# KamilSJaron/smudgeplot

Hardware: NVIDIA H100
Metric: k-mers/sec scanned (hetmers) at 1/2/4/8 H100; bit-exact .smu vs ref C (higher is better)
Workload: dtype u64

## Files before the change

smudgeplot_b200/csrc/hm_symm.cu:

```cuda
#include <cuda_runtime.h>
#include <stdint.h>
#include <stdio.h>
#include <stdlib.h>
#include <string.h>

#include "hetmers_b200.h"
#include "hm_internal.h"
#include "hm_device.cuh"

#define RS_THREADS 256
#define RS_EPT     8
#define RS_TILE    (RS_THREADS*RS_EPT)
#define RS_HALO    64
#define RS_WIN     (RS_TILE+2*RS_HALO)
#define RS_SCANCAP RS_HALO
#define RS_RUNCAP  (RS_HALO+1)
#define RS_LONGRUN 32
#ifndef RS_MINBLOCKS
#define RS_MINBLOCKS 5
#endif
#ifndef RS_STAGE
#define RS_STAGE   384
#endif

#define SY_STATUS_ASYMMETRIC 1ull
#define SY_STATUS_OVERFLOW   2ull

#define SY_HDR_CAND   0
#define SY_HDR_STATUS 1
#define SY_HDR_RUNS   2
#define SY_HDR_S      3
#define SY_HDR_PEND   4
#define SY_HDR_QUERY  5

struct SymmView
  { unsigned long long *cand_n;
    unsigned long long *status;
    uint32_t *bloom;
    uint32_t  seg_words;
    int       n_seg, self;
    uint64_t  first_key[HM_MAX_SHARDS];
    uint64_t *cand_key, *cand_lo, *cand_meta;
    unsigned long long cand_cap;
    unsigned long long *runs_n;
    uint64_t *runs;
    unsigned long long runs_cap;
    uint64_t *s_key, *s_lo;
    unsigned long long s_cap;
    const hm_stream_sview *sviews;
    uint64_t *pend, *pend_key, *pend_lo;
    uint64_t *q_key, *q_lo, *q_tag;
    unsigned long long pend_cap, q_cap;
  };

template <int KW>
__device__ __forceinline__ void bloom_slot(const SymmView &W, int seg, int kmer, uint64_t hi, uint64_t lo,
                                           uint32_t *&word, uint32_t &mask)
{ const int Pr = kmer >> 1, pup = kmer-Pr;
  uint64_t sfx;
  if (KW == 1)
    sfx = hi >> (64-2*kmer);
  else
    { const int sr = 128-2*kmer;
      sfx = sr == 0 ? lo : ((lo >> sr) | (hi << (64-sr)));
    }
  if (2*Pr < 64)
    sfx &= (((uint64_t) 1 << (2*Pr)) - 1);
  const uint64_t pfx = hi >> (64-2*pup);
  uint32_t h = ((uint32_t) sfx ^ (uint32_t) (sfx >> 32) * 0x85EBCA6Bu) * 0x9E3779B1u;
  uint32_t g = ((uint32_t) pfx ^ (uint32_t) (pfx >> 32) * 0xC2B2AE35u) * 0x27D4EB2Fu;
  h ^= h >> 15;
  word = W.bloom + (size_t) seg * W.seg_words + __umulhi(h * 0x2C1B3C6Du,W.seg_words);
  mask = (1u << (g >> 27)) | (1u << ((g >> 22) & 31));
}

__device__ __forceinline__ uint32_t ld_keep(const uint32_t *p)
{ uint32_t v; uint64_t pol;
  asm volatile("createpolicy.fractional.L2::evict_last.b64 %0, 1.0;" : "=l"(pol));
  asm volatile("ld.global.nc.L1::no_allocate.L2::cache_hint.u32 %0, [%1], %2;" : "=r"(v) : "l"(p), "l"(pol));
  return v;
}

__device__ __forceinline__ uint64_t ld_stream(const uint64_t *p)
{ uint64_t v, pol;
  asm volatile("createpolicy.fractional.L2::evict_first.b64 %0, 1.0;" : "=l"(pol));
  asm volatile("ld.global.nc.L1::no_allocate.L2::cache_hint.u64 %0, [%1], %2;" : "=l"(v) : "l"(p), "l"(pol));
  return v;
}

__device__ __forceinline__ int owner_of(const SymmView &W, uint64_t hi)
{ int r = 0;
  for (int s = 1; s < W.n_seg; s++)
    r += (hi >= W.first_key[s]);
  return r;
}

template <typename IdxT, int KW>
__device__ __noinline__ void neighbours_slow(const uint64_t *__restrict__ keys, const uint64_t *__restrict__ keys_lo,
                                             const uint16_t *__restrict__ cnt, const IdxT *__restrict__ bucket,
                                             int bshift, int kmer, int p0, int pup,
                                             uint64_t x, uint64_t xl, int cx,
                                             int &H, int &U, int64_t &part, int &ppos)
{ H = 0; U = 0; part = -1; ppos = 0;
  for (int p = p0; p < kmer; p++)
    { int b = base_at<KW>(x,xl,p);
      for (int c = 0; c < 4; c++)
        { if (c == b) continue;
          uint64_t y = x, yl = xl;
          set_base<KW>(y,yl,p,c);
          int64_t j = bucket_find<IdxT,KW>(keys,keys_lo,bucket,bshift,y,yl);
          if (j >= 0 && cx + (int) __ldg(cnt+j) <= HM_SMAX)
            { H += 1;
              if (p >= pup) U += 1;
              part = j; ppos = p;
            }
        }
    }
}


__device__ __forceinline__ uint64_t fp_mix(uint64_t hi, uint64_t lo, uint32_t c, uint64_t seed)
{ uint64_t v = (hi ^ seed) * 0xBF58476D1CE4E5B9ull;
  v ^= v >> 32;
  v = (v + lo + ((uint64_t) c << 40) + c) * 0x94D049BB133111EBull;
  v ^= v >> 29;
  v *= (seed | 1);
  v ^= v >> 32;
  return v;
}

template <int KW>
__global__ void __launch_bounds__(256)
symm_fingerprint_kernel(const uint64_t *__restrict__ keys, const uint64_t *__restrict__ keys_lo,
                        const uint16_t *__restrict__ cnt, int64_t i0, int64_t i1, int kmer,
                        uint64_t seed0, uint64_t seed1, unsigned long long *__restrict__ acc)
{ uint64_t a0 = 0, a1 = 0, a2 = 0, a3 = 0;
// ... 79 lines not shown
  out->off_cand_meta = at;  at += 8*cap;
  out->cand_cap = cap;
  out->off_runs = at;       out->runs_cap = range/3 + 1024;   at += 8*out->runs_cap;
  out->n_seg = n_seg;
  out->range = range;
  out->bytes = (at+255) & ~255ll;
  return HM_OK;
}

static void bloom_window(cudaStream_t st, const void *base, size_t bytes, int on)
{ static int limit_set[64] = {0};
  static size_t max_win[64] = {0}, max_persist[64] = {0};
  int dev = 0;
  cudaGetDevice(&dev);
  if (dev < 0 || dev >= 64) return;
  if (!limit_set[dev])
    { cudaDeviceProp p;
      limit_set[dev] = 1;
      if (cudaGetDeviceProperties(&p,dev) == cudaSuccess)
        { max_win[dev] = (size_t) p.accessPolicyMaxWindowSize;
          max_persist[dev] = (size_t) p.persistingL2CacheMaxSize;
          if (max_persist[dev] > 0)
            cudaDeviceSetLimit(cudaLimitPersistingL2CacheSize,max_persist[dev]);
        }
      cudaGetLastError();
    }
  if (max_win[dev] == 0 || max_persist[dev] == 0)
    return;
  cudaStreamAttrValue a;
  memset(&a,0,sizeof(a));
  if (on)
    { size_t w = bytes < max_win[dev] ? bytes : max_win[dev];
      a.accessPolicyWindow.base_ptr  = (void *) base;
      a.accessPolicyWindow.num_bytes = w;
      a.accessPolicyWindow.hitRatio  = w <= max_persist[dev] ? 1.0f : (float) max_persist[dev] / (float) w;
      a.accessPolicyWindow.hitProp   = cudaAccessPropertyPersisting;
      a.accessPolicyWindow.missProp  = cudaAccessPropertyStreaming;
    }
  cudaStreamSetAttribute(st,cudaStreamAttributeAccessPolicyWindow,&a);
  cudaGetLastError();
}

static int l2_persist(void)
{ const char *e = getenv("HETMERS_L2_PERSIST");
  return (e == NULL || strcmp(e,"0") != 0);
}

static SymmView make_view(void *d_work, const hm_symm_layout *L, const hm_symm_shards *sh)
{ SymmView W;
  uint8_t *b = (uint8_t *) d_work;
  memset(&W,0,sizeof(W));
  W.cand_n    = (unsigned long long *) (b + L->off_header) + SY_HDR_CAND;
  W.status    = W.cand_n + SY_HDR_STATUS;
  W.bloom     = (uint32_t *) (b + L->off_bloom);
  W.seg_words = (uint32_t) L->seg_words;
  W.n_seg     = L->n_seg;
  W.self      = 0;
  if (sh != NULL && sh->n_seg > 1)
    { W.self = sh->self;
      for (int r = 0; r < sh->n_seg; r++) W.first_key[r] = sh->first_key[r];
    }
  W.cand_key  = (uint64_t *) (b + L->off_cand_key);
  W.cand_lo   = (uint64_t *) (b + L->off_cand_lo);
  W.cand_meta = (uint64_t *) (b + L->off_cand_meta);
  W.cand_cap  = (unsigned long long) L->cand_cap;
  W.runs_n    = W.cand_n + SY_HDR_RUNS;
  W.runs      = (uint64_t *) (b + L->off_runs);
  W.runs_cap  = (unsigned long long) L->runs_cap;
  return W;
}


template <int KW> struct RsSmem
  { uint64_t *key, *klo;
    uint16_t *cnt;
    uint64_t *ckey, *clo, *cmeta;
    uint16_t *t1;
    uint16_t *t2r;
  };

__device__ __forceinline__ uint64_t pack_meta(int cx, int cy, int pos, int yb)
{ return (uint64_t) cx | ((uint64_t) cy << 16) | ((uint64_t) pos << 32) | ((uint64_t) yb << 40); }

template <int KW>
__device__ __forceinline__ void stage_candidates(const RsSmem<KW> &S, unsigned *s_nc, const SymmView &W,
                                                 bool emit, uint64_t x, uint64_t xl, uint64_t meta,
                                                 int lane, unsigned lt)
{ const unsigned bal = __ballot_sync(0xffffffffu,emit);
  if (bal == 0)
    return;
  unsigned base = 0;
  if (lane == 0)
    base = atomicAdd(s_nc,(unsigned) __popc(bal));
  base = __shfl_sync(0xffffffffu,base,0);
  const unsigned at = base + __popc(bal & lt);
  const bool     over = emit && (at >= RS_STAGE);
  if (emit && !over)
    { S.ckey[at] = x;
      if (KW == 2) S.clo[at] = xl;
      S.cmeta[at] = meta;
    }
  if (base + __popc(bal) <= RS_STAGE)
    return;
  const unsigned ob = __ballot_sync(0xffffffffu,over);
  unsigned long long g0 = 0;
  if (lane == 0)
    g0 = atomicAdd(W.cand_n,(unsigned long long) __popc(ob));
  g0 = __shfl_sync(0xffffffffu,g0,0) + (unsigned long long) __popc(ob & lt);
  if (over)
    { if (g0 < W.cand_cap)
        { W.cand_key[g0] = x;
          if (KW == 2) W.cand_lo[g0] = xl;
          W.cand_meta[g0] = meta;
        }
      else
        atomicOr(W.status,SY_STATUS_OVERFLOW);
    }
}

template <int KW>
__device__ __forceinline__ void s_push(const SymmView &W, uint64_t x, uint64_t xl)
{ const unsigned m = __activemask();
  const int      lane = threadIdx.x & 31, lead = __ffs(m)-1;
  unsigned long long at = 0;
  if (lane == lead)
    at = atomicAdd(W.cand_n + SY_HDR_S,(unsigned long long) __popc(m));
  at = __shfl_sync(m,at,lead) + (unsigned long long) __popc(m & ((1u << lane)-1));
  if (at < W.s_cap)
    { W.s_key[at] = x;
      if (KW == 2) W.s_lo[at] = xl;
    }
  else
    atomicOr(W.status,SY_STATUS_OVERFLOW);
}

template <int KW, bool SL>
__device__ __forceinline__ void bloom_insert(const SymmView &W, int kmer, uint64_t x, uint64_t xl)
{ uint32_t *word, mask;
  bloom_slot<KW>(W,W.self,kmer,x,xl,word,mask);
  atomicOr(word,mask);
  if (SL)
    s_push<KW>(W,x,xl);
}

template <typename IdxT, int KW, bool SL>
__global__ void __launch_bounds__(256)
runs_kernel(const uint64_t *__restrict__ keys, const uint64_t *__restrict__ keys_lo,
            const uint16_t *__restrict__ cnt, int64_t n, const IdxT *__restrict__ bucket, int bshift,
            int kmer, int64_t lo, int64_t hi, const SymmView W)
{ const int      Pr = kmer >> 1, pup = kmer-Pr, psh = 64-2*Pr;
  const uint64_t pmask = ~(uint64_t) 0 << psh;
  const unsigned FULL = 0xffffffffu;
  const int      lane = threadIdx.x & 31;
  const unsigned lt   = (1u << lane) - 1;
  unsigned long long nrl = *W.runs_n;
  if (nrl > W.runs_cap) nrl = W.runs_cap;
  const int64_t nr     = (int64_t) nrl;
  const int64_t stride = (int64_t) gridDim.x * blockDim.x;
  for (int64_t r0 = (int64_t) blockIdx.x * blockDim.x + threadIdx.x - lane; r0 < nr; r0 += stride)
    { const int64_t r = r0+lane;
      const bool    valid = (r < nr);
      int64_t  h = 0;
      uint64_t x0 = 0;
      if (valid)
        { h  = (int64_t) W.runs[r];
          x0 = __ldg(keys+h);
        }
      unsigned lb = __ballot_sync(FULL,valid);
      while (lb != 0)
        { const int     src = __ffs(lb)-1;
          lb &= lb-1;
          const int64_t hh = __shfl_sync(FULL,h,src);
          const uint64_t xx = __shfl_sync(FULL,x0,src);
          int64_t end = hh+1;
          while (true)
            { const int64_t t = end+lane;
              const bool same = (t < n) && (((__ldg(keys+t) ^ xx) & pmask) == 0);
              const unsigned sb = __ballot_sync(FULL,same);
              if (sb == FULL) { end += 32; continue; }
              end += __ffs(~sb)-1;
              break;
            }
          for (int64_t g0 = hh; g0 < end; g0 += 32)
            { const int64_t g = g0+lane;
              bool     emit = false;
              uint64_t x = 0, xl = 0, meta = 0;
              if (g < end && g >= lo && g < hi)
                { x = __ldg(keys+g);
                  if (KW == 2) xl = __ldg(keys_lo+g);
                  const int cx = __ldg(cnt+g);
                  int Hn, Un, ppos; int64_t part;
                  neighbours_slow<IdxT,KW>(keys,keys_lo,cnt,bucket,bshift,kmer,Pr,pup,x,xl,cx,Hn,Un,part,ppos);
                  if (Un > 0)
                    bloom_insert<KW,SL>(W,kmer,x,xl);
                  if (Hn == 1 && part > g)
                    { const uint64_t y = __ldg(keys+part), yl = KW == 2 ? __ldg(keys_lo+part) : 0;
                      const int cy = __ldg(cnt+part);
                      int Hy, Uy, py; int64_t party;
                      neighbours_slow<IdxT,KW>(keys,keys_lo,cnt,bucket,bshift,kmer,Pr,pup,y,yl,cy,Hy,Uy,party,py);
                      if (Hy == 1)
                        { emit = true;
                          meta = pack_meta(cx,cy,ppos,base_at<KW>(y,yl,ppos));
                        }
                    }
                }
              const unsigned eb = __ballot_sync(FULL,emit);
              if (eb != 0)
                { unsigned long long base = 0;
                  if (lane == 0)
                    base = atomicAdd(W.cand_n,(unsigned long long) __popc(eb));
                  base = __shfl_sync(FULL,base,0) + (unsigned long long) __popc(eb & lt);
                  if (emit)
                    { if (base < W.cand_cap)
                        { W.cand_key[base] = x;
                          if (KW == 2) W.cand_lo[base] = xl;
                          W.cand_meta[base] = meta;
                        }
                      else
                        atomicOr(W.status,SY_STATUS_OVERFLOW);
                    }
                }
            }
        }
    }
}
// ... 18 lines not shown
}

template <int KW, bool SL, int LMAX>
__device__ __forceinline__ bool settle_members(const RsSmem<KW> &S, const SymmView &W, int kmer, int Pr, int pup,
                                               int h, int L, int a, bool in, bool own, int lane,
                                               uint64_t &x, uint64_t &xl, uint64_t &meta)
{ int Hx = 0, Ux = 0, part = 0, ppos = 0, cx = 0;
  if (in)
    { x  = S.key[h+a];
      xl = KW == 2 ? S.klo[h+a] : 0;
      cx = S.cnt[h+a];
      auto mate = [&](int b)
        { int pos;
          if (b < L && b != a && one_base_in_run(run_sfx<KW>(x ^ S.key[h+b],KW == 2 ? xl ^ S.klo[h+b] : 0,Pr),Pr,pos) &&
              cx + (int) S.cnt[h+b] <= HM_SMAX)
            { Hx += 1;
              if (pos >= pup) Ux += 1;
              part = b; ppos = pos;
            }
        };
      if constexpr (LMAX > 0)
        {
#pragma unroll
          for (int b = 0; b < LMAX; b++)
            mate(b);
        }
      else
        for (int b = 0; b < L; b++)
          mate(b);
      if (own && Ux > 0)
        bloom_insert<KW,SL>(W,kmer,x,xl);
    }
  const int pl = lane + part - a;
  int       Hy = __shfl_sync(0xffffffffu,Hx,pl & 31);
  if (!in || !own || Hx != 1 || part < a)
    return false;
  const uint64_t y = S.key[h+part], yl = KW == 2 ? S.klo[h+part] : 0;
  const int      cy = S.cnt[h+part];
  if (pl > 31)
    { Hy = 0;
      for (int b = 0; b < L; b++)
        { int pos;
          if (b != part && one_base_in_run(run_sfx<KW>(y ^ S.key[h+b],KW == 2 ? yl ^ S.klo[h+b] : 0,Pr),Pr,pos) &&
              cy + (int) S.cnt[h+b] <= HM_SMAX)
            Hy += 1;
        }
    }
  if (Hy != 1)
    return false;
  meta = pack_meta(cx,cy,ppos,base_at<KW>(y,yl,ppos));
  return true;
}

#ifdef RS_PROBE
#define RS_PHASES 6
#define RS_PROBE_SLOTS 1024
__device__ unsigned long long rs_probe_cycles[RS_PROBE_SLOTS*RS_PHASES];
__device__ int rs_probe_mode;
#define RS_PROBE_TILE(b)  (rs_probe_mode == 2 ? (b) % 64 : (b))
#define RS_PROBE_START    long long rs_t = clock64(); unsigned long long rs_acc[RS_PHASES] = {0, 0, 0, 0, 0, 0};
#define RS_PROBE_MARK(ph) { const long long t_ = clock64(); rs_acc[ph] += (unsigned long long) (t_ - rs_t); rs_t = t_; }
#define RS_PROBE_FLUSH()  { if (lane == 0) _Pragma("unroll") for (int p_ = 0; p_ < RS_PHASES; p_++) \
                              atomicAdd(rs_probe_cycles + (blockIdx.x % RS_PROBE_SLOTS)*RS_PHASES + p_,rs_acc[p_]); }
#define RS_PROBE_LOADONLY() if (rs_probe_mode == 1) { RS_PROBE_FLUSH(); return; }

extern "C" int hm_probe_runscan(int mode, unsigned long long *cycles)
{ static unsigned long long rows[RS_PROBE_SLOTS*RS_PHASES];
  cudaError_t e = cudaDeviceSynchronize();
  if (e == cudaSuccess && cycles != NULL)
    { e = cudaMemcpyFromSymbol(rows,rs_probe_cycles,sizeof(rows));
      for (int p = 0; p < RS_PHASES; p++)
        { cycles[p] = 0;
          for (int r = 0; r < RS_PROBE_SLOTS; r++)
            cycles[p] += rows[r*RS_PHASES+p];
        }
    }
  memset(rows,0,sizeof(rows));
  if (e == cudaSuccess)
    e = cudaMemcpyToSymbol(rs_probe_cycles,rows,sizeof(rows));
  if (e == cudaSuccess)
    e = cudaMemcpyToSymbol(rs_probe_mode,&mode,sizeof(mode));
  return e == cudaSuccess ? HM_OK : hm_cuda_fail(e,"hm_probe_runscan");
}
#else
#define RS_PROBE_TILE(b)  (b)
#define RS_PROBE_START
#define RS_PROBE_MARK(ph)
#define RS_PROBE_FLUSH()
#define RS_PROBE_LOADONLY()
#endif

template <typename IdxT, int KW, bool SL>
__global__ void __launch_bounds__(RS_THREADS,RS_MINBLOCKS)
runscan_kernel(const uint64_t *__restrict__ keys, const uint64_t *__restrict__ keys_lo,
               const uint16_t *__restrict__ cnt, int64_t n, const IdxT *__restrict__ bucket, int bshift,
               int kmer, int64_t lo, int64_t hi, int64_t tile0, int use_tma, const SymmView W)
{ extern __shared__ __align__(128) uint8_t smem[];
  __shared__ __align__(8) uint64_t s_bar;
  __shared__ unsigned s_nc, s_nr, s_done;
  RsSmem<KW> S;
  S.key   = (uint64_t *) smem;
  S.klo   = S.key + (KW == 2 ? RS_WIN : 0);
  S.ckey  = S.key + KW*RS_WIN;
  S.clo   = S.ckey + (KW == 2 ? RS_STAGE : 0);
  S.cmeta = S.ckey + KW*RS_STAGE;
  S.cnt   = (uint16_t *) (S.cmeta + RS_STAGE);
  S.t1    = S.cnt + RS_WIN;
  S.t2r   = S.t1 + RS_TILE/2;

  const int      Pr   = kmer >> 1;
  const int      pup  = kmer - Pr;
  const int      psh  = 64-2*Pr;
  const uint64_t pmask = ~(uint64_t) 0 << psh;
  const unsigned FULL = 0xffffffffu;
  const int      lane = threadIdx.x & 31;
  const int      warp = threadIdx.x >> 5;
  const unsigned lt   = (1u << lane) - 1;
  RS_PROBE_START

  const int64_t T0 = (tile0 + RS_PROBE_TILE(blockIdx.x)) * RS_TILE;
  const int64_t ws = T0 - RS_HALO;
  const int64_t e0 = ws > 0 ? ws : 0;
  const int64_t e1 = T0+RS_TILE+RS_HALO < n ? T0+RS_TILE+RS_HALO : n;
  const int     v0 = (int) (e0-ws), v1 = (int) (e1-ws);

  const int m   = v1-v0;
  const int mt  = use_tma ? (m & ~7) : 0;
  if (threadIdx.x == 0)
    { s_nc = 0; s_nr = 0; s_done = 0;
      if (mt > 0)
        { mbar_init(&s_bar,1);
          fence_proxy_async_smem();
        }
    }
  __syncthreads();
  if (threadIdx.x == 0 && mt > 0)
    { mbar_arrive_expect_tx(&s_bar,(unsigned) (mt*(8*KW+2)));
      bulk_copy_g2s(S.key+v0,keys+e0,(unsigned) (8*mt),&s_bar);
      if (KW == 2)
        bulk_copy_g2s(S.klo+v0,keys_lo+e0,(unsigned) (8*mt),&s_bar);
      bulk_copy_g2s(S.cnt+v0,cnt+e0,(unsigned) (2*mt),&s_bar);
    }
  if (mt < m || v0 > 0 || v1 < RS_WIN)
    { for (int j = mt + threadIdx.x; j < m; j += RS_THREADS)
        { S.key[v0+j] = keys[e0+j];
          if (KW == 2) S.klo[v0+j] = keys_lo[e0+j];
          S.cnt[v0+j] = cnt[e0+j];
        }
      if (mt > 0)
        mbar_wait(&s_bar,0);
      __syncthreads();
      const uint64_t sa = ~S.key[v0], sb = ~S.key[v1-1];
      __syncthreads();
      for (int j = threadIdx.x; j < RS_WIN; j += RS_THREADS)
        if (j < v0)       S.key[j] = sa;
        else if (j >= v1) S.key[j] = sb;
      __syncthreads();
    }
  else
    mbar_wait(&s_bar,0);
  RS_PROBE_MARK(0)
  RS_PROBE_LOADONLY()

  const int wd0 = RS_HALO/32 + warp*RS_EPT;
  unsigned  eqw = 0;
#pragma unroll
  for (int t = 0; t < RS_EPT+2; t++)
    { const int i = (wd0-1+t)*32 + lane;
      bool eq;
      if (psh >= 32)
        { const uint32_t a = (uint32_t) (S.key[i] >> 32);
          uint32_t       b = __shfl_down_sync(FULL,a,1);
          if (lane == 31) b = (uint32_t) (S.key[i+1] >> 32);
          eq = (((a ^ b) >> (psh-32)) == 0);
        }
      else
        eq = (((S.key[i] ^ S.key[i+1]) & pmask) == 0);
      const unsigned bal = __ballot_sync(FULL,eq);
      if (lane == t) eqw = bal;
    }
  RS_PROBE_MARK(1)

  const int a0 = RS_HALO + (lo > T0 ? (int) (lo-T0 < RS_TILE ? lo-T0 : RS_TILE) : 0);
  const int a1 = RS_HALO + (hi-T0 < RS_TILE ? (int) (hi-T0) : RS_TILE);
  uint16_t *my1  = S.t1  + warp*(RS_TILE/2/(RS_THREADS/32));
  int n1, n3;
  { const unsigned P = __shfl_up_sync(FULL,eqw,1), N = __shfl_down_sync(FULL,eqw,1);
    unsigned m2 = 0, m3 = 0;
    const int wd = wd0-1+lane;
    if (lane >= 1 && lane <= RS_EPT)
      { const unsigned E = eqw;
        const unsigned em1 = (E << 1) | (P >> 31);
        const unsigned em2 = (E << 2) | (P >> 30);
        const unsigned ep1 = (E >> 1) | (N << 31);
        const int      s0  = wd*32;
        unsigned act = 0xffffffffu;
        if (s0 < a0)      act &= (a0-s0 >= 32) ? 0u : (0xffffffffu << (a0-s0));
        if (s0+32 > a1)   act &= (a1-s0 <= 0)  ? 0u : (0xffffffffu >> (s0+32-a1));
        const unsigned more = (em1 & E) | (E & ep1) | (em1 & em2);
        m2 = (E & ~em1 & ~ep1) & act;
        m3 = more & act & ~em1;
      }
    const int c2 = __popc(m2), c3 = __popc(m3);
    int pre2 = c2, pre3 = c3;
#pragma unroll
    for (int o = 1; o <= RS_EPT; o <<= 1)
      { int v2 = __shfl_up_sync(FULL,pre2,o), v3 = __shfl_up_sync(FULL,pre3,o);
        if (lane >= o) { pre2 += v2; pre3 += v3; }
      }
    n1 = __shfl_sync(FULL,pre2,RS_EPT);
    n3 = __shfl_sync(FULL,pre3,RS_EPT);
    int at = pre2-c2;
    while (m2 != 0)
      { my1[at++] = (uint16_t) (wd*32 + __ffs(m2)-1);
        m2 &= m2-1;
      }
    at = n1 + pre3-c3;
    while (m3 != 0)
      { my1[at++] = (uint16_t) (wd*32 + __ffs(m3)-1);
        m3 &= m3-1;
      }
  }
  __syncwarp();
  RS_PROBE_MARK(2)

  for (int i0 = 0; i0 < n1; i0 += 32)
    { const int i = i0+lane;
      bool     emit = false;
      uint64_t x = 0, xl = 0, meta = 0;
      if (i < n1)
        { const int w = my1[i];
          x = S.key[w];
          const uint64_t y = S.key[w+1];
          uint64_t yl = 0;
          if (KW == 2) { xl = S.klo[w]; yl = S.klo[w+1]; }
          const int cx = S.cnt[w], cy = S.cnt[w+1];
          int pos;
          if (one_base_in_run(run_sfx<KW>(x ^ y,xl ^ yl,Pr),Pr,pos) && cx+cy <= HM_SMAX)
            { emit = true;
              meta = pack_meta(cx,cy,pos,base_at<KW>(y,yl,pos));
              if (pos >= pup)
                { bloom_insert<KW,SL>(W,kmer,x,xl);
                  bloom_insert<KW,SL>(W,kmer,y,yl);
                }
            }
        }
      stage_candidates<KW>(S,&s_nc,W,emit,x,xl,meta,lane,lt);
    }
  RS_PROBE_MARK(3)

  const int b1 = hi-T0 < RS_TILE+RS_HALO ? RS_HALO + (int) (hi-T0) : RS_WIN;
  for (int i0 = 0; i0 < n3; i0 += 32)
    { const int i = i0+lane;
      const int h = i < n3 ? my1[n1+i] : 0;
      int       L = 0;
      {
        const int      t  = (h >> 5) - (wd0-1);
        const unsigned w0 = __shfl_sync(FULL,eqw,t & 31), w1 = __shfl_sync(FULL,eqw,(t+1) & 31);
        const unsigned up = __funnelshift_r(w0,w1,h & 31);
        if (i < n3)
          L = (~up != 0) ? __ffs((int) ~up) : 33;
      }
      const int Ls = L <= 8 ? L : 0;
      int inc = Ls;
#pragma unroll
      for (int o = 1; o < 32; o <<= 1)
        { const int v = __shfl_up_sync(FULL,inc,o);
          if (lane >= o) inc += v;
        }
      const int M = __shfl_sync(FULL,inc,31);
      for (int t0 = 0; t0 < M; t0 += 32)
        { const int t = t0+lane;
          int r = 0;
#pragma unroll
          for (int s = 16; s > 0; s >>= 1)
            if (__shfl_sync(FULL,inc,r+s-1) <= t) r += s;
          const int hr = __shfl_sync(FULL,h,r), Lr = __shfl_sync(FULL,Ls,r);
          const int a  = t - (__shfl_sync(FULL,inc,r) - Lr);
          bool     emit = false;
          uint64_t x = 0, xl = 0, meta = 0;
          emit = settle_members<KW,SL,8>(S,W,kmer,Pr,pup,hr,Lr,a,t < M,hr+a < b1,lane,x,xl,meta);
          stage_candidates<KW>(S,&s_nc,W,emit,x,xl,meta,lane,lt);
        }
      unsigned lb = __ballot_sync(FULL,L > 8);
      while (lb != 0)
        { const int src = __ffs(lb)-1;
          lb &= lb-1;
          const int hh = __shfl_sync(FULL,h,src);
          int       LL = __shfl_sync(FULL,L,src);
          if (LL > 32)
            { const uint64_t xh = S.key[hh];
              while (LL <= RS_RUNCAP)
                { const int      t = hh+LL+lane;
                  const unsigned sb = __ballot_sync(FULL,t < RS_WIN && ((S.key[t] ^ xh) & pmask) == 0);
                  if (sb != FULL) { LL += __ffs(~sb)-1; break; }
                  LL += 32;
                }
            }
          if (LL > RS_RUNCAP || hh+LL >= RS_WIN)
            { if (lane == 0)
                S.t2r[atomicAdd(&s_nr,1u)] = (uint16_t) hh;
              continue;
            }
          for (int a0 = 0; a0 < LL; a0 += 32)
            { const int a = a0+lane;
              bool     emit = false;
              uint64_t x = 0, xl = 0, meta = 0;
              emit = settle_members<KW,SL,0>(S,W,kmer,Pr,pup,hh,LL,a,a < LL,hh+a < b1,lane,x,xl,meta);
              stage_candidates<KW>(S,&s_nc,W,emit,x,xl,meta,lane,lt);
            }
        }
    }
  RS_PROBE_MARK(4)

  __syncwarp();
  unsigned last = 0;
  if (lane == 0)
    { __threadfence_block();
      last = (atomicAdd(&s_done,1u) == RS_THREADS/32-1);
    }
  last = __shfl_sync(FULL,last,0);
  if (!last)
    { RS_PROBE_MARK(5) RS_PROBE_FLUSH() return; }
  __threadfence_block();
  const unsigned nr = s_nr;
  if (nr > 0)
    { unsigned long long rb = 0;
      if (lane == 0)
        rb = atomicAdd(W.runs_n,(unsigned long long) nr);
      rb = __shfl_sync(FULL,rb,0);
      for (unsigned i = lane; i < nr; i += 32)
        if (rb+i < W.runs_cap)
          W.runs[rb+i] = (uint64_t) (T0 + ((int) S.t2r[i] - RS_HALO));
        else
          atomicOr(W.status,SY_STATUS_OVERFLOW);
    }
  const unsigned nc = s_nc < RS_STAGE ? s_nc : RS_STAGE;
  if (nc == 0)
    { RS_PROBE_MARK(5) RS_PROBE_FLUSH() return; }
  unsigned long long base = 0;
  if (lane == 0)
    base = atomicAdd(W.cand_n,(unsigned long long) nc);
  base = __shfl_sync(FULL,base,0);
  for (unsigned i = lane; i < nc; i += 32)
    { unsigned long long at = base + i;
      if (at < W.cand_cap)
        { W.cand_key[at] = S.ckey[i];
          if (KW == 2) W.cand_lo[at] = S.clo[i];
          W.cand_meta[at] = S.cmeta[i];
        }
      else
        atomicOr(W.status,SY_STATUS_OVERFLOW);
    }
  RS_PROBE_MARK(5)
  RS_PROBE_FLUSH()
}

template <typename IdxT, int KW, bool SL>
__global__ void __launch_bounds__(RS_THREADS,RS_MINBLOCKS)
runscan_dense_kernel(const uint64_t *__restrict__ keys, const uint64_t *__restrict__ keys_lo,
                     const uint16_t *__restrict__ cnt, int64_t n, int kmer, int64_t lo, int64_t hi,
                     int64_t tile0, int use_tma, const SymmView W)
{ extern __shared__ __align__(128) uint8_t smem[];
  __shared__ __align__(8) uint64_t s_bar;
  __shared__ unsigned s_nc, s_nl, s_done;
  __shared__ unsigned s_eq[RS_WIN/32+1];
  RsSmem<KW> S;
  S.key   = (uint64_t *) smem;
  S.klo   = S.key + (KW == 2 ? RS_WIN : 0);
  S.ckey  = S.key + KW*RS_WIN;
  S.clo   = S.ckey + (KW == 2 ? RS_STAGE : 0);
  S.cmeta = S.ckey + KW*RS_STAGE;
  S.cnt   = (uint16_t *) (S.cmeta + RS_STAGE);
  S.t1    = S.cnt + RS_WIN;
  S.t2r   = S.t1 + RS_WIN;
  uint16_t *s_part = S.t2r + RS_TILE/8;
  unsigned *hu = (unsigned *) (s_part + RS_WIN);
  uint32_t *rem = hu + RS_WIN/2;

  const int      Pr   = kmer >> 1, pup = kmer - Pr, psh = 64-2*Pr;
  const uint64_t pmask = ~(uint64_t) 0 << psh;
  const unsigned FULL = 0xffffffffu;
  const int      lane = threadIdx.x & 31;
  const int      warp = threadIdx.x >> 5;
  const unsigned lt   = (1u << lane) - 1;

  const int64_t T0 = (tile0 + blockIdx.x) * RS_TILE;
  const int64_t ws = T0 - RS_HALO;
  const int64_t e0 = ws > 0 ? ws : 0;
  const int64_t e1 = T0+RS_TILE+RS_HALO < n ? T0+RS_TILE+RS_HALO : n;
  const int     v0 = (int) (e0-ws), v1 = (int) (e1-ws);

  const int m   = v1-v0;
  const int mt  = use_tma ? (m & ~7) : 0;
  if (threadIdx.x == 0)
    { s_nc = 0; s_nl = 0; s_done = 0;
      if (mt > 0)
        { mbar_init(&s_bar,1);
          fence_proxy_async_smem();
        }
    }
  for (int j = threadIdx.x; j < RS_WIN/2; j += RS_THREADS)
    hu[j] = 0;
  __syncthreads();
  if (threadIdx.x == 0 && mt > 0)
    { mbar_arrive_expect_tx(&s_bar,(unsigned) (mt*(8*KW+2)));
      bulk_copy_g2s(S.key+v0,keys+e0,(unsigned) (8*mt),&s_bar);
      if (KW == 2)
        bulk_copy_g2s(S.klo+v0,keys_lo+e0,(unsigned) (8*mt),&s_bar);
      bulk_copy_g2s(S.cnt+v0,cnt+e0,(unsigned) (2*mt),&s_bar);
    }
  if (mt < m || v0 > 0 || v1 < RS_WIN)
    { for (int j = mt + threadIdx.x; j < m; j += RS_THREADS)
        { S.key[v0+j] = keys[e0+j];
          if (KW == 2) S.klo[v0+j] = keys_lo[e0+j];
          S.cnt[v0+j] = cnt[e0+j];
        }
      if (mt > 0)
        mbar_wait(&s_bar,0);
      __syncthreads();
// ... 25 lines not shown
  __syncthreads();

  const int a0 = RS_HALO + (lo > T0 ? (int) (lo-T0 < RS_TILE ? lo-T0 : RS_TILE) : 0);
  const int a1 = RS_HALO + (hi-T0 < RS_TILE ? (int) (hi-T0) : RS_TILE);
  for (int i = threadIdx.x; i < RS_WIN; i += RS_THREADS)
    { const int      w = i >> 5, b = i & 31;
      const unsigned up = __funnelshift_r(s_eq[w],s_eq[w+1],b);
      const int      fwd = (~up == 0) ? 32 : __ffs((int) ~up)-1;
      int back = 0;
      if (i > 0)
        { const int      wq = (i-1) >> 5, bq = (i-1) & 31;
          const unsigned dn = __funnelshift_l(wq > 0 ? s_eq[wq-1] : 0u,s_eq[wq],31-bq);
          back = (~dn == 0) ? 32 : __clz((int) ~dn);
        }
      uint16_t mark = (uint16_t) fwd;
      if (back+fwd+1 > RS_LONGRUN)
        { mark = 0xffff;
          if (back == 0 && i >= a0 && i < a1)
            S.t2r[atomicAdd(&s_nl,1u)] = (uint16_t) i;
        }
      S.t1[i] = mark;
      s_part[i] = (uint16_t) i;
    }
  __syncthreads();

  for (int i = threadIdx.x; i < RS_WIN; i += RS_THREADS)
    { const int fwd = S.t1[i];
      if (fwd == 0 || fwd == 0xffff)
        continue;
      const int cx = S.cnt[i];
      if (narrow)
        { const uint32_t rx = rem[i];
          for (int j = i+1; j <= i+fwd; j++)
            { const uint32_t d = rx ^ rem[j];
              const uint32_t u = (d | (d>>1)) & 0x55555555u;
              if ((u & (u-1)) == 0 && cx + (int) S.cnt[j] <= HM_SMAX)
                { const int      pos = Pr + (__clz((int) d) >> 1);
                  const unsigned inc = 1u | (pos >= pup ? 0x100u : 0u);
                  atomicAdd(hu + (i>>1), inc << (16*(i&1)));
                  atomicAdd(hu + (j>>1), inc << (16*(j&1)));
                  s_part[i] = (uint16_t) j;
                  s_part[j] = (uint16_t) i;
                }
            }
        }
      else
        { const uint64_t x = S.key[i], xl = KW == 2 ? S.klo[i] : 0;
          for (int j = i+1; j <= i+fwd; j++)
            { int pos;
              if (one_base_apart<KW>(x,xl,S.key[j],KW == 2 ? S.klo[j] : 0,pos) && cx + (int) S.cnt[j] <= HM_SMAX)
                { const unsigned inc = 1u | (pos >= pup ? 0x100u : 0u);
                  atomicAdd(hu + (i>>1), inc << (16*(i&1)));
                  atomicAdd(hu + (j>>1), inc << (16*(j&1)));
                  s_part[i] = (uint16_t) j;
                  s_part[j] = (uint16_t) i;
                }
            }
        }
    }
  __syncthreads();

  for (int i0 = RS_HALO + (threadIdx.x & ~31); i0 < RS_HALO+RS_TILE; i0 += RS_THREADS)
    { const int i = i0+lane;
      bool     emit = false;
      uint64_t x = 0, xl = 0, meta = 0;
      if (i >= a0 && i < a1 && S.t1[i] != 0xffff)
        { const unsigned c = (hu[i>>1] >> (16*(i&1))) & 0xffffu;
          const int H = (int) (c & 0xff), U = (int) (c >> 8);
          if (H > 0)
            { x = S.key[i];
              if (KW == 2) xl = S.klo[i];
              if (U > 0)
                bloom_insert<KW,SL>(W,kmer,x,xl);
              const int j = s_part[i];
              if (H == 1 && j > i && ((hu[j>>1] >> (16*(j&1))) & 0xffu) == 1)
                { const uint64_t y = S.key[j], yl = KW == 2 ? S.klo[j] : 0;
                  int pos;
                  one_base_apart<KW>(x,xl,y,yl,pos);
                  emit = true;
                  meta = pack_meta(S.cnt[i],S.cnt[j],pos,base_at<KW>(y,yl,pos));
                }
            }
        }
      stage_candidates<KW>(S,&s_nc,W,emit,x,xl,meta,lane,lt);
    }

  __syncwarp();
  unsigned last = 0;
  if (lane == 0)
    { __threadfence_block();
      last = (atomicAdd(&s_done,1u) == RS_THREADS/32-1);
    }
  last = __shfl_sync(FULL,last,0);
  if (!last)
    return;
  __threadfence_block();
  const unsigned nr = s_nl;
  if (nr > 0)
    { unsigned long long rb = 0;
      if (lane == 0)
        rb = atomicAdd(W.runs_n,(unsigned long long) nr);
      rb = __shfl_sync(FULL,rb,0);
      for (unsigned i = lane; i < nr; i += 32)
        if (rb+i < W.runs_cap)
          W.runs[rb+i] = (uint64_t) (T0 + ((int) S.t2r[i] - RS_HALO));
        else
          atomicOr(W.status,SY_STATUS_OVERFLOW);
    }
  const unsigned nc = s_nc < RS_STAGE ? s_nc : RS_STAGE;
  if (nc == 0)
    return;
  unsigned long long base = 0;
  if (lane == 0)
    base = atomicAdd(W.cand_n,(unsigned long long) nc);
  base = __shfl_sync(FULL,base,0);
  for (unsigned i = lane; i < nc; i += 32)
    { unsigned long long at = base + i;
      if (at < W.cand_cap)
        { W.cand_key[at] = S.ckey[i];
          if (KW == 2) W.cand_lo[at] = S.clo[i];
          W.cand_meta[at] = S.cmeta[i];
        }
      else
        atomicOr(W.status,SY_STATUS_OVERFLOW);
    }
}

template <typename I, int K> struct Inst { typedef I IdxT; static constexpr int KW = K; };

template <class F>
static cudaError_t dispatch(int kmer, int idx64, F f)
{ if (kmer <= 32)
    return idx64 ? f(Inst<uint64_t,1>()) : f(Inst<uint32_t,1>());
  return idx64 ? f(Inst<uint64_t,2>()) : f(Inst<uint32_t,2>());
}

template <typename IdxT, int KW, bool SL = false>
static cudaError_t launch_runscan(const uint64_t *keys, const uint64_t *keys_lo, const uint16_t *cnt, int64_t n,
                                  const void *bucket, int bits, int kmer, int64_t lo, int64_t hi,
                                  const SymmView &W, cudaStream_t st)
{ static int configured[64] = {0};
  int dev = 0;
  cudaGetDevice(&dev);
  int64_t tile0 = lo/RS_TILE, tile1 = (hi+RS_TILE-1)/RS_TILE;
  int     tma   = ((((uintptr_t) keys) | ((uintptr_t) cnt) | ((uintptr_t) (keys_lo ? keys_lo : keys))) & 15) == 0;
  const int   Pr  = kmer >> 1;
  double      lam = (2*Pr >= 62) ? 0.0 : (double) n / (double) ((uint64_t) 1 << (2*Pr));
  bool        dense = (lam > 0.6);
  const char *force = getenv("HETMERS_RUNSCAN");
  if (force != NULL && strcmp(force,"dense") == 0)  dense = true;
  if (force != NULL && strcmp(force,"sparse") == 0) dense = false;
  cudaError_t e;
  if (dense)
    { size_t smem = (size_t) RS_WIN*(8*KW+2) + (size_t) RS_STAGE*8*(KW+1) +
                    2*(size_t) (RS_WIN+RS_TILE/8+RS_WIN) + 4*(size_t) (RS_WIN/2+RS_WIN);
      if (smem > 48*1024 && (dev >= 64 || !(configured[dev] & 2)))
        { e = cudaFuncSetAttribute(runscan_dense_kernel<IdxT,KW,SL>,cudaFuncAttributeMaxDynamicSharedMemorySize,(int) smem);
          if (e != cudaSuccess) return e;
          if (dev < 64) configured[dev] |= 2;
        }
      runscan_dense_kernel<IdxT,KW,SL><<<(unsigned) (tile1-tile0),RS_THREADS,smem,st>>>
          (keys,keys_lo,cnt,n,kmer,lo,hi,tile0,tma,W);
    }
  else
    { size_t smem = (size_t) RS_WIN*(8*KW+2) + (size_t) RS_STAGE*8*(KW+1) +
                    2*(size_t) (RS_TILE/2+RS_TILE/2);
      if (smem > 48*1024 && (dev >= 64 || !(configured[dev] & 1)))
        { e = cudaFuncSetAttribute(runscan_kernel<IdxT,KW,SL>,cudaFuncAttributeMaxDynamicSharedMemorySize,(int) smem);
          if (e != cudaSuccess) return e;
          if (dev < 64) configured[dev] |= 1;
        }
      runscan_kernel<IdxT,KW,SL><<<(unsigned) (tile1-tile0),RS_THREADS,smem,st>>>
          (keys,keys_lo,cnt,n,(const IdxT *) bucket,64-bits,kmer,lo,hi,tile0,tma,W);
    }
  return cudaGetLastError();
}

template <typename IdxT, int KW, bool SL = false>
static cudaError_t launch_runs(const uint64_t *keys, const uint64_t *keys_lo, const uint16_t *cnt, int64_t n,
                               const void *bucket, int bits, int kmer, int64_t lo, int64_t hi,
                               const SymmView &W, cudaStream_t st)
{
  int dev = 0, sms = 132;
  cudaGetDevice(&dev);
  cudaDeviceGetAttribute(&sms,cudaDevAttrMultiProcessorCount,dev);
  int64_t want = ((hi-lo)/64+255)/256;
  int     grid = (int) (want < sms*8 ? (want > 0 ? want : 1) : sms*8);
  runs_kernel<IdxT,KW,SL><<<grid,256,0,st>>>(keys,keys_lo,cnt,n,(const IdxT *) bucket,64-bits,kmer,lo,hi,W);
  return cudaGetLastError();
}

extern "C" int hm_k_symm_runscan(const uint64_t *d_keys, const uint64_t *d_keys_lo, const uint16_t *d_cnt, int64_t n,
                                 const void *d_bucket, int bits, int idx64, int kmer, int64_t lo, int64_t hi,
                                 void *d_work, const hm_symm_layout *layout, const hm_symm_shards *shards,
                                 void *stream)
{ if (kmer < HM_SYMM_MIN_KMER || kmer > HM_MAX_KMER)
    return hm_set_error(HM_EUNSUPPORTED,"symmetric scan needs %d <= k <= %d (k=%d)",HM_SYMM_MIN_KMER,HM_MAX_KMER,kmer);
  if (lo < 0 || hi > n || lo > hi || bits < 1 || bits > 30 || d_work == NULL || layout == NULL)
    return hm_set_error(HM_EINVAL,"symm_runscan: bad range [%lld,%lld) of %lld or bits %d",
                        (long long) lo,(long long) hi,(long long) n,bits);
  if ((kmer > 32) != (d_keys_lo != NULL))
    return hm_set_error(HM_EINVAL,"symm_runscan: second key word array %s for k=%d",
                        d_keys_lo ? "given" : "missing",kmer);
  if ((shards != NULL && shards->n_seg > 1) != (layout->n_seg > 1) ||
      (shards != NULL && shards->n_seg > 1 && (shards->n_seg != layout->n_seg || shards->self < 0 ||
                                               shards->self >= shards->n_seg)))
    return hm_set_error(HM_EINVAL,"symm_runscan: shard table does not match the work-area layout");
  cudaStream_t st = (cudaStream_t) stream;
  SymmView W = make_view(d_work,layout,shards);
  HM_CUDA(cudaMemsetAsync(W.cand_n,0,256,st));
  HM_CUDA(cudaMemsetAsync(W.bloom + (size_t) W.self*W.seg_words,0,sizeof(uint32_t)*(size_t) W.seg_words,st));
  if (l2_persist())
    bloom_window(st,W.bloom,sizeof(uint32_t)*(size_t) W.seg_words*(size_t) W.n_seg,1);
  if (hi == lo)
    return HM_OK;
  cudaError_t e = dispatch(kmer,idx64,[&](auto I)
    { return launch_runscan<typename decltype(I)::IdxT,decltype(I)::KW>(d_keys,d_keys_lo,d_cnt,n,d_bucket,bits,kmer,
                                                                       lo,hi,W,st); });
  if (e != cudaSuccess)
    return hm_cuda_fail(e,"runscan_kernel");
  return HM_OK;
}

extern "C" int hm_k_symm_runs(const uint64_t *d_keys, const uint64_t *d_keys_lo, const uint16_t *d_cnt, int64_t n,
                              const void *d_bucket, int bits, int idx64, int kmer, int64_t lo, int64_t hi,
                              void *d_work, const hm_symm_layout *layout, const hm_symm_shards *shards,
                              void *stream)
{ if (kmer < HM_SYMM_MIN_KMER || kmer > HM_MAX_KMER || d_work == NULL || layout == NULL ||
      (kmer > 32) != (d_keys_lo != NULL) || lo < 0 || hi > n || lo > hi)
    return hm_set_error(HM_EINVAL,"symm_runs: bad arguments");
  if (hi == lo)
    return HM_OK;
  cudaStream_t st = (cudaStream_t) stream;
  SymmView W = make_view(d_work,layout,shards);
  cudaError_t e = dispatch(kmer,idx64,[&](auto I)
    { return launch_runs<typename decltype(I)::IdxT,decltype(I)::KW>(d_keys,d_keys_lo,d_cnt,n,d_bucket,bits,kmer,
                                                                    lo,hi,W,st); });
  if (e != cudaSuccess)
    return hm_cuda_fail(e,"runs_kernel");
  return HM_OK;
}


#define RV_TS   192
#define RV_TM   96
#define RV_TROW 97
#define RV_THREADS 1024
#ifndef RV_ILP
#define RV_ILP 2
#endif
#define RV_QCAP  (32*(RV_ILP+1))
#define RV_PROBE 4
#define RV_HA    (1ull << 48)
#define RV_HB    (1ull << 49)

// ... 879 lines not shown
```

Before: 119.3 billion.

## Decouple sparse runscan geometry and trim per-run settle and bloom work

Gives the sparse runscan kernel its own tile geometry: 12 elements per thread, 4 min blocks, a staging area sized to the tile and a smaller run-list buffer. The bloom hash is split so a pair of inserts computes the prefix mask once and reuses it for both words. Run groups whose runs are all short settle through the 4-wide path instead of the 8-wide one. Larger tiles amortize halo loads per block but need more shared memory and registers per block, which may lower occupancy.

```diff
diff --git a/smudgeplot_b200/csrc/hm_symm.cu b/smudgeplot_b200/csrc/hm_symm.cu
--- a/smudgeplot_b200/csrc/hm_symm.cu
+++ b/smudgeplot_b200/csrc/hm_symm.cu
@@ -22,6 +22,26 @@
 #ifndef RS_STAGE
 #define RS_STAGE   384
 #endif
+
+#ifndef RSS_EPT
+#define RSS_EPT       12
+#endif
+#ifndef RSS_THREADS
+#define RSS_THREADS   256
+#endif
+#ifndef RSS_MINBLOCKS
+#define RSS_MINBLOCKS 4
+#endif
+#define RSS_TILE      (RSS_THREADS*RSS_EPT)
+#define RSS_WIN       (RSS_TILE+2*RS_HALO)
+#define RSS_LISTED    (RSS_TILE/64+2)
+#ifndef RSS_STAGE
+#define RSS_STAGE     (RSS_TILE/8)
+#endif
+static_assert(RSS_EPT >= 1 && RSS_EPT+2 <= 32, "runscan_kernel: a warp's words and its two halo words are one per lane");
+static_assert(RSS_THREADS % 32 == 0 && RSS_THREADS >= 32 && RSS_THREADS <= 1024, "runscan_kernel: whole warps");
+static_assert(RSS_WIN+1 <= 65536, "runscan_kernel: window slots are 16-bit task-list entries");
+static_assert(RSS_STAGE >= 32, "runscan_kernel: a staging area of at least one warp's records");
 
 #define SY_STATUS_ASYMMETRIC 1ull
 #define SY_STATUS_OVERFLOW   2ull
@@ -52,6 +72,30 @@
     uint64_t *q_key, *q_lo, *q_tag;
     unsigned long long pend_cap, q_cap;
   };
+
+template <int KW>
+__device__ __forceinline__ uint32_t *bloom_word(const SymmView &W, int seg, int kmer, uint64_t hi, uint64_t lo)
+{ const int Pr = kmer >> 1;
+  uint64_t sfx;
+  if (KW == 1)
+    sfx = hi >> (64-2*kmer);
+  else
+    { const int sr = 128-2*kmer;
+      sfx = sr == 0 ? lo : ((lo >> sr) | (hi << (64-sr)));
+    }
+  if (2*Pr < 64)
+    sfx &= (((uint64_t) 1 << (2*Pr)) - 1);
+  uint32_t h = ((uint32_t) sfx ^ (uint32_t) (sfx >> 32) * 0x85EBCA6Bu) * 0x9E3779B1u;
+  h ^= h >> 15;
+  return W.bloom + (size_t) seg * W.seg_words + __umulhi(h * 0x2C1B3C6Du,W.seg_words);
+}
+
+__device__ __forceinline__ uint32_t bloom_mask(int kmer, uint64_t hi)
+{ const int      pup = kmer - (kmer >> 1);
+  const uint64_t pfx = hi >> (64-2*pup);
+  const uint32_t g = ((uint32_t) pfx ^ (uint32_t) (pfx >> 32) * 0xC2B2AE35u) * 0x27D4EB2Fu;
+  return (1u << (g >> 27)) | (1u << ((g >> 22) & 31));
+}
 
 template <int KW>
 __device__ __forceinline__ void bloom_slot(const SymmView &W, int seg, int kmer, uint64_t hi, uint64_t lo,
@@ -297,7 +341,7 @@
 __device__ __forceinline__ uint64_t pack_meta(int cx, int cy, int pos, int yb)
 { return (uint64_t) cx | ((uint64_t) cy << 16) | ((uint64_t) pos << 32) | ((uint64_t) yb << 40); }
 
-template <int KW>
+template <int KW, int STAGE>
 __device__ __forceinline__ void stage_candidates(const RsSmem<KW> &S, unsigned *s_nc, const SymmView &W,
                                                  bool emit, uint64_t x, uint64_t xl, uint64_t meta,
                                                  int lane, unsigned lt)
@@ -309,13 +353,13 @@
     base = atomicAdd(s_nc,(unsigned) __popc(bal));
   base = __shfl_sync(0xffffffffu,base,0);
   const unsigned at = base + __popc(bal & lt);
-  const bool     over = emit && (at >= RS_STAGE);
+  const bool     over = emit && (at >= STAGE);
   if (emit && !over)
     { S.ckey[at] = x;
       if (KW == 2) S.clo[at] = xl;
       S.cmeta[at] = meta;
     }
-  if (base + __popc(bal) <= RS_STAGE)
+  if (base + __popc(bal) <= STAGE)
     return;
   const unsigned ob = __ballot_sync(0xffffffffu,over);
   unsigned long long g0 = 0;
@@ -356,6 +400,18 @@
   atomicOr(word,mask);
   if (SL)
     s_push<KW>(W,x,xl);
+}
+
+template <int KW, bool SL>
+__device__ __forceinline__ void bloom_insert_pair(const SymmView &W, int kmer, uint64_t x, uint64_t xl,
+                                                  uint64_t y, uint64_t yl)
+{ const uint32_t mask = bloom_mask(kmer,x);
+  atomicOr(bloom_word<KW>(W,W.self,kmer,x,xl),mask);
+  atomicOr(bloom_word<KW>(W,W.self,kmer,y,yl),mask);
+  if (SL)
+    { s_push<KW>(W,x,xl);
+      s_push<KW>(W,y,yl);
+    }
 }
 
 template <typename IdxT, int KW, bool SL>
@@ -540,6 +596,9 @@
     e = cudaMemcpyToSymbol(rs_probe_mode,&mode,sizeof(mode));
   return e == cudaSuccess ? HM_OK : hm_cuda_fail(e,"hm_probe_runscan");
 }
+
+extern "C" void hm_probe_runscan_geometry(int *out)
+{ out[0] = RSS_THREADS; out[1] = RSS_EPT; out[2] = RSS_MINBLOCKS; out[3] = RSS_STAGE; }
 #else
 #define RS_PROBE_TILE(b)  (b)
 #define RS_PROBE_START
@@ -549,7 +608,7 @@
 #endif
 
 template <typename IdxT, int KW, bool SL>
-__global__ void __launch_bounds__(RS_THREADS,RS_MINBLOCKS)
+__global__ void __launch_bounds__(RSS_THREADS,RSS_MINBLOCKS)
 runscan_kernel(const uint64_t *__restrict__ keys, const uint64_t *__restrict__ keys_lo,
                const uint16_t *__restrict__ cnt, int64_t n, const IdxT *__restrict__ bucket, int bshift,
                int kmer, int64_t lo, int64_t hi, int64_t tile0, int use_tma, const SymmView W)
@@ -558,13 +617,13 @@
   __shared__ unsigned s_nc, s_nr, s_done;
   RsSmem<KW> S;
   S.key   = (uint64_t *) smem;
-  S.klo   = S.key + (KW == 2 ? RS_WIN : 0);
-  S.ckey  = S.key + KW*RS_WIN;
-  S.clo   = S.ckey + (KW == 2 ? RS_STAGE : 0);
-  S.cmeta = S.ckey + KW*RS_STAGE;
-  S.cnt   = (uint16_t *) (S.cmeta + RS_STAGE);
-  S.t1    = S.cnt + RS_WIN;
-  S.t2r   = S.t1 + RS_TILE/2;
+  S.klo   = S.key + (KW == 2 ? RSS_WIN : 0);
+  S.ckey  = S.key + KW*RSS_WIN;
+  S.clo   = S.ckey + (KW == 2 ? RSS_STAGE : 0);
+  S.cmeta = S.ckey + KW*RSS_STAGE;
+  S.cnt   = (uint16_t *) (S.cmeta + RSS_STAGE);
+  S.t1    = S.cnt + RSS_WIN;
+  S.t2r   = S.t1 + RSS_TILE/2;
 
   const int      Pr   = kmer >> 1;
   const int      pup  = kmer - Pr;
@@ -576,10 +635,10 @@
   const unsigned lt   = (1u << lane) - 1;
   RS_PROBE_START
 
-  const int64_t T0 = (tile0 + RS_PROBE_TILE(blockIdx.x)) * RS_TILE;
+  const int64_t T0 = (tile0 + RS_PROBE_TILE(blockIdx.x)) * RSS_TILE;
   const int64_t ws = T0 - RS_HALO;
   const int64_t e0 = ws > 0 ? ws : 0;
-  const int64_t e1 = T0+RS_TILE+RS_HALO < n ? T0+RS_TILE+RS_HALO : n;
+  const int64_t e1 = T0+RSS_TILE+RS_HALO < n ? T0+RSS_TILE+RS_HALO : n;
   const int     v0 = (int) (e0-ws), v1 = (int) (e1-ws);
 
   const int m   = v1-v0;
@@ -599,8 +658,8 @@
         bulk_copy_g2s(S.klo+v0,keys_lo+e0,(unsigned) (8*mt),&s_bar);
       bulk_copy_g2s(S.cnt+v0,cnt+e0,(unsigned) (2*mt),&s_bar);
     }
-  if (mt < m || v0 > 0 || v1 < RS_WIN)
-    { for (int j = mt + threadIdx.x; j < m; j += RS_THREADS)
+  if (mt < m || v0 > 0 || v1 < RSS_WIN)
+    { for (int j = mt + threadIdx.x; j < m; j += RSS_THREADS)
         { S.key[v0+j] = keys[e0+j];
           if (KW == 2) S.klo[v0+j] = keys_lo[e0+j];
           S.cnt[v0+j] = cnt[e0+j];
@@ -610,7 +669,7 @@
       __syncthreads();
       const uint64_t sa = ~S.key[v0], sb = ~S.key[v1-1];
       __syncthreads();
-      for (int j = threadIdx.x; j < RS_WIN; j += RS_THREADS)
+      for (int j = threadIdx.x; j < RSS_WIN; j += RSS_THREADS)
         if (j < v0)       S.key[j] = sa;
         else if (j >= v1) S.key[j] = sb;
       __syncthreads();
@@ -620,10 +679,10 @@
   RS_PROBE_MARK(0)
   RS_PROBE_LOADONLY()
 
-  const int wd0 = RS_HALO/32 + warp*RS_EPT;
+  const int wd0 = RS_HALO/32 + warp*RSS_EPT;
   unsigned  eqw = 0;
 #pragma unroll
-  for (int t = 0; t < RS_EPT+2; t++)
+  for (int t = 0; t < RSS_EPT+2; t++)
     { const int i = (wd0-1+t)*32 + lane;
       bool eq;
       if (psh >= 32)
@@ -639,14 +698,14 @@
     }
   RS_PROBE_MARK(1)
 
-  const int a0 = RS_HALO + (lo > T0 ? (int) (lo-T0 < RS_TILE ? lo-T0 : RS_TILE) : 0);
-  const int a1 = RS_HALO + (hi-T0 < RS_TILE ? (int) (hi-T0) : RS_TILE);
-  uint16_t *my1  = S.t1  + warp*(RS_TILE/2/(RS_THREADS/32));
+  const int a0 = RS_HALO + (lo > T0 ? (int) (lo-T0 < RSS_TILE ? lo-T0 : RSS_TILE) : 0);
+  const int a1 = RS_HALO + (hi-T0 < RSS_TILE ? (int) (hi-T0) : RSS_TILE);
+  uint16_t *my1  = S.t1  + warp*(RSS_EPT*16);
   int n1, n3;
   { const unsigned P = __shfl_up_sync(FULL,eqw,1), N = __shfl_down_sync(FULL,eqw,1);
     unsigned m2 = 0, m3 = 0;
     const int wd = wd0-1+lane;
-    if (lane >= 1 && lane <= RS_EPT)
+    if (lane >= 1 && lane <= RSS_EPT)
       { const unsigned E = eqw;
         const unsigned em1 = (E << 1) | (P >> 31);
         const unsigned em2 = (E << 2) | (P >> 30);
@@ -662,12 +721,12 @@
     const int c2 = __popc(m2), c3 = __popc(m3);
     int pre2 = c2, pre3 = c3;
 #pragma unroll
-    for (int o = 1; o <= RS_EPT; o <<= 1)
+    for (int o = 1; o <= RSS_EPT; o <<= 1)
       { int v2 = __shfl_up_sync(FULL,pre2,o), v3 = __shfl_up_sync(FULL,pre3,o);
         if (lane >= o) { pre2 += v2; pre3 += v3; }
       }
-    n1 = __shfl_sync(FULL,pre2,RS_EPT);
-    n3 = __shfl_sync(FULL,pre3,RS_EPT);
+    n1 = __shfl_sync(FULL,pre2,RSS_EPT);
+    n3 = __shfl_sync(FULL,pre3,RSS_EPT);
     int at = pre2-c2;
     while (m2 != 0)
       { my1[at++] = (uint16_t) (wd*32 + __ffs(m2)-1);
@@ -698,16 +757,14 @@
             { emit = true;
               meta = pack_meta(cx,cy,pos,base_at<KW>(y,yl,pos));
               if (pos >= pup)
-                { bloom_insert<KW,SL>(W,kmer,x,xl);
-                  bloom_insert<KW,SL>(W,kmer,y,yl);
-                }
+                bloom_insert_pair<KW,SL>(W,kmer,x,xl,y,yl);
             }
         }
-      stage_candidates<KW>(S,&s_nc,W,emit,x,xl,meta,lane,lt);
+      stage_candidates<KW,RSS_STAGE>(S,&s_nc,W,emit,x,xl,meta,lane,lt);
     }
   RS_PROBE_MARK(3)
 
-  const int b1 = hi-T0 < RS_TILE+RS_HALO ? RS_HALO + (int) (hi-T0) : RS_WIN;
+  const int b1 = hi-T0 < RSS_TILE+RS_HALO ? RS_HALO + (int) (hi-T0) : RSS_WIN;
   for (int i0 = 0; i0 < n3; i0 += 32)
     { const int i = i0+lane;
       const int h = i < n3 ? my1[n1+i] : 0;
@@ -737,8 +794,11 @@
           const int a  = t - (__shfl_sync(FULL,inc,r) - Lr);
           bool     emit = false;
           uint64_t x = 0, xl = 0, meta = 0;
-          emit = settle_members<KW,SL,8>(S,W,kmer,Pr,pup,hr,Lr,a,t < M,hr+a < b1,lane,x,xl,meta);
-          stage_candidates<KW>(S,&s_nc,W,emit,x,xl,meta,lane,lt);
+          if (__any_sync(FULL,t < M && Lr > 4))
+            emit = settle_members<KW,SL,8>(S,W,kmer,Pr,pup,hr,Lr,a,t < M,hr+a < b1,lane,x,xl,meta);
+          else
+            emit = settle_members<KW,SL,4>(S,W,kmer,Pr,pup,hr,Lr,a,t < M,hr+a < b1,lane,x,xl,meta);
+          stage_candidates<KW,RSS_STAGE>(S,&s_nc,W,emit,x,xl,meta,lane,lt);
         }
       unsigned lb = __ballot_sync(FULL,L > 8);
       while (lb != 0)
@@ -750,12 +810,12 @@
             { const uint64_t xh = S.key[hh];
               while (LL <= RS_RUNCAP)
                 { const int      t = hh+LL+lane;
-                  const unsigned sb = __ballot_sync(FULL,t < RS_WIN && ((S.key[t] ^ xh) & pmask) == 0);
+                  const unsigned sb = __ballot_sync(FULL,t < RSS_WIN && ((S.key[t] ^ xh) & pmask) == 0);
                   if (sb != FULL) { LL += __ffs(~sb)-1; break; }
                   LL += 32;
                 }
             }
-          if (LL > RS_RUNCAP || hh+LL >= RS_WIN)
+          if (LL > RS_RUNCAP || hh+LL >= RSS_WIN)
             { if (lane == 0)
                 S.t2r[atomicAdd(&s_nr,1u)] = (uint16_t) hh;
               continue;
@@ -765,7 +825,7 @@
               bool     emit = false;
               uint64_t x = 0, xl = 0, meta = 0;
               emit = settle_members<KW,SL,0>(S,W,kmer,Pr,pup,hh,LL,a,a < LL,hh+a < b1,lane,x,xl,meta);
-              stage_candidates<KW>(S,&s_nc,W,emit,x,xl,meta,lane,lt);
+              stage_candidates<KW,RSS_STAGE>(S,&s_nc,W,emit,x,xl,meta,lane,lt);
             }
         }
     }
@@ -775,7 +835,7 @@
   unsigned last = 0;
   if (lane == 0)
     { __threadfence_block();
-      last = (atomicAdd(&s_done,1u) == RS_THREADS/32-1);
+      last = (atomicAdd(&s_done,1u) == RSS_THREADS/32-1);
     }
   last = __shfl_sync(FULL,last,0);
   if (!last)
@@ -793,7 +853,7 @@
         else
           atomicOr(W.status,SY_STATUS_OVERFLOW);
     }
-  const unsigned nc = s_nc < RS_STAGE ? s_nc : RS_STAGE;
+  const unsigned nc = s_nc < RSS_STAGE ? s_nc : RSS_STAGE;
   if (nc == 0)
     { RS_PROBE_MARK(5) RS_PROBE_FLUSH() return; }
   unsigned long long base = 0;
@@ -985,7 +1045,7 @@
                 }
             }
         }
-      stage_candidates<KW>(S,&s_nc,W,emit,x,xl,meta,lane,lt);
+      stage_candidates<KW,RS_STAGE>(S,&s_nc,W,emit,x,xl,meta,lane,lt);
     }
 
   __syncwarp();
@@ -1045,7 +1105,6 @@
 { static int configured[64] = {0};
   int dev = 0;
   cudaGetDevice(&dev);
-  int64_t tile0 = lo/RS_TILE, tile1 = (hi+RS_TILE-1)/RS_TILE;
   int     tma   = ((((uintptr_t) keys) | ((uintptr_t) cnt) | ((uintptr_t) (keys_lo ? keys_lo : keys))) & 15) == 0;
   const int   Pr  = kmer >> 1;
   double      lam = (2*Pr >= 62) ? 0.0 : (double) n / (double) ((uint64_t) 1 << (2*Pr));
@@ -1055,7 +1114,8 @@
   if (force != NULL && strcmp(force,"sparse") == 0) dense = false;
   cudaError_t e;
   if (dense)
-    { size_t smem = (size_t) RS_WIN*(8*KW+2) + (size_t) RS_STAGE*8*(KW+1) +
+    { const int64_t tile0 = lo/RS_TILE, tile1 = (hi+RS_TILE-1)/RS_TILE;
+      size_t smem = (size_t) RS_WIN*(8*KW+2) + (size_t) RS_STAGE*8*(KW+1) +
                     2*(size_t) (RS_WIN+RS_TILE/8+RS_WIN) + 4*(size_t) (RS_WIN/2+RS_WIN);
       if (smem > 48*1024 && (dev >= 64 || !(configured[dev] & 2)))
         { e = cudaFuncSetAttribute(runscan_dense_kernel<IdxT,KW,SL>,cudaFuncAttributeMaxDynamicSharedMemorySize,(int) smem);
@@ -1066,14 +1126,15 @@
           (keys,keys_lo,cnt,n,kmer,lo,hi,tile0,tma,W);
     }
   else
-    { size_t smem = (size_t) RS_WIN*(8*KW+2) + (size_t) RS_STAGE*8*(KW+1) +
-                    2*(size_t) (RS_TILE/2+RS_TILE/2);
+    { const int64_t tile0 = lo/RSS_TILE, tile1 = (hi+RSS_TILE-1)/RSS_TILE;
+      size_t smem = (size_t) RSS_WIN*(8*KW+2) + (size_t) RSS_STAGE*8*(KW+1) +
+                    2*(size_t) (RSS_TILE/2+RSS_LISTED);
       if (smem > 48*1024 && (dev >= 64 || !(configured[dev] & 1)))
         { e = cudaFuncSetAttribute(runscan_kernel<IdxT,KW,SL>,cudaFuncAttributeMaxDynamicSharedMemorySize,(int) smem);
           if (e != cudaSuccess) return e;
           if (dev < 64) configured[dev] |= 1;
         }
-      runscan_kernel<IdxT,KW,SL><<<(unsigned) (tile1-tile0),RS_THREADS,smem,st>>>
+      runscan_kernel<IdxT,KW,SL><<<(unsigned) (tile1-tile0),RSS_THREADS,smem,st>>>
           (keys,keys_lo,cnt,n,(const IdxT *) bucket,64-bits,kmer,lo,hi,tile0,tma,W);
     }
   return cudaGetLastError();
```

After: 120.6 billion (median of 6 runs). 1.01x the previous value.
